# lukebeddow/gripper-mujoco

Hardware: AMD Instinct MI355X
Metric: env-steps/sec (batched rollout) at 4096 envs; obs max-rel-err vs C++ ref (higher is better)
Workload: dtype f64; 1 GPU; C3: set6_synthetic 20 mixed objects, randomised spawn (object drawn per episode, spawn_into_scene grid search on the device), steady state: envs staggered over episode steps 1..250 by an untimed pre-roll, benchmark mix (1 episode in 4: the closed-loop grasp-lift-hold program; otherwise the scripted grasp mix: close / squeeze / palm / lift + jitter), canonical sensor/reward config, device auto-rese; envs_per_gpu=4096, global_envs=4096, parallelism=env-shard x1, substeps_per_env_step=63

## Files before the change

__graft_entry__.py:

```python
from __future__ import annotations

import os
import subprocess
import sys

REPO = os.path.dirname(os.path.abspath(__file__))
PKG = os.path.join(REPO, "gripper-mujoco_amd")


def build() -> None:
    if PKG not in sys.path:
        sys.path.insert(0, PKG)
    from gmx.build import build as build_lib
    build_lib(verbose=True)
    subprocess.run(["make", "-s", "-C", os.path.join(REPO, "oracle"), os.path.join(REPO, "oracle", "liboracle.so")],
                   check=True)
    if os.path.isdir("/root/reference/src"):
        subprocess.run(["make", "-s", "-C", os.path.join(REPO, "oracle"), "ref"], check=True)
    import gmx
    gmx.load_library()


def smoke() -> None:
    import numpy as np
    if PKG not in sys.path:
        sys.path.insert(0, PKG)
    sys.path.insert(0, os.path.join(REPO, "tests"))
    import torch
    assert torch.cuda.is_available(), "smoke() needs a GPU"
    import gmx
    import oracle_lib
    s = gmx.canonical_settings(noise=False, seed=5)
    env = gmx.BatchedGripperEnv(2, object_set="set1_synthetic", settings=s, seed=5, device=0)
    sp = env.make_spawn(x=[0.06, 0.07], y=[0.06, 0.07], idx=0)
    obs0 = env.reset(spawn=sp)
    orc = []
    for e in range(2):
        o = oracle_lib.OracleEnv(env.model, env.cfg, env.objects, e)
        o.reset(sp[e])
        orc.append(o)
        assert np.allclose(obs0[e], o.observation(), atol=1e-5), "reset observation differs from oracle"
    rng = np.random.default_rng(1234)
    for t in range(3):
        a = rng.uniform(-1, 1, size=(2, env.n_actions)).astype(np.float32)
        obs, rew, term, trunc = env.step(a)
        for e in range(2):
            ro, rr, rd = orc[e].step(a[e])
            ro = np.asarray(ro, dtype=np.float64)
            d = np.abs(obs[e] - ro)
            big = np.abs(ro) >= 1e-3
            rel = float((d[big] / np.abs(ro[big])).max()) if big.any() else 0.0
            assert rel <= 1e-4 and float(d[~big].max(initial=0)) <= 1e-4, \
                f"step {t} env {e}: obs rel err {rel:.3e} vs oracle"
            assert bool(term[e]) == bool(rd), "done flag differs from oracle"
            assert abs(float(rew[e]) - float(rr)) <= 1e-5 + 1e-4 * abs(float(rr)), "reward differs from oracle"
    env.close()
    print("smoke ok: 2 envs x 3 env-steps match the oracle")


if __name__ == "__main__":
    build()
    if len(sys.argv) > 1 and sys.argv[1] == "smoke":
        smoke()
```

gripper-mujoco_amd/csrc/gm_newton.hip:

```cpp

#pragma once
#include "gm_rows.h"
#include "gm_newton_point.h"

GM_PHYSICS_BEGIN
template <int CL>
__device__ void smooth_matvec(SharedT<CL>& S, const GmTopo* __restrict__ T, const real* v, real* out, int lane) {
  if (lane < T->nv) {
    const int d = lane, c = T->dof_grp[d], p = T->dof_p[d];
    real acc;
    if (c >= 0 && c < 3) {
      const real* H = S.Hf[c];
      const int f0 = T->dof_f0[c];
      acc = H[TRI(p, 0)] * v[T->dof_base];
#pragma unroll
      for (int j = 1; j <= CL; j++) {
        const real hv = H[(j <= p) ? TRI(p, j) : TRI(j, p)];
        acc = acc + hv * v[f0 + j - 1];
      }
    } else if (c == GM_GRP_BASE) {
      acc = S.Hbb * v[T->dof_base];
#pragma unroll
      for (int f = 0; f < 3; f++)
#pragma unroll
        for (int q = 1; q <= CL; q++) acc = acc + S.Hf[f][TRI(q, 0)] * v[T->dof_f0[f] + q - 1];
      acc = acc + S.Hp[TRI(1, 0)] * v[T->dof_palm];
    } else if (c == GM_GRP_PALM) {
      acc = S.Hp[TRI(1, 0)] * v[T->dof_base] + S.Hp[TRI(1, 1)] * v[T->dof_palm];
    } else {
      acc = 0;
#pragma unroll
      for (int l = 0; l < 6; l++) {
        const real hv = S.Ho[(l <= p) ? TRI(p, l) : TRI(l, p)];
        acc = acc + hv * v[T->dof_obj + l];
      }
    }
    out[d] = acc;
  }
  GM_WAVE_SYNC();
}

struct LineSearch { real alpha; bool capped; };
__device__ __forceinline__ LineSearch line_search(int lane, int ncon, int nl, const RowsT& R, const real* jq, real jql,
                                                  const real* dj, real djl, real g0, real h0, int& nls) {
  const bool clane = lane < ncon;
  real alpha = 1.0, lo = 0.0, hi = 0.0;
  bool hi_set = false, newton = false, have_prev = false;
  unsigned prev = 0;
  int ls = 0;
  for (; ls < GM_NEWTON_MAXLS; ls++) {
    nls++;
    unsigned pat = 0;
    real tg[4], th[4];
#pragma unroll
    for (int e = 0; e < 4; e++) {
      const real j = jq[e] + alpha * dj[e];
      const bool a = clane && j < 0;
      pat |= (unsigned)a << e;
      tg[e] = a ? (R.cD * j) * dj[e] : 0.0;
      th[e] = a ? (R.cD * dj[e]) * dj[e] : 0.0;
    }
    const real jl = jql + alpha * djl;
    const real tgl = (R.lD * jl) * djl, thl = (R.lD * djl) * djl;
    const bool same_piece = have_prev && __ballot(pat != prev) == 0ull;
    if (newton && same_piece) break;
    const real g = (g0 + alpha * h0) + row_sum(lane, ncon, nl, tg, tgl);
    const real hh = h0 + row_sum(lane, ncon, nl, th, thl);
    if (g == 0.0) break;
    if (g < 0) lo = alpha; else { hi = alpha; hi_set = true; }
    if (!(hh > 0)) break;
    real an = alpha - div_n(g, hh);
    newton = true;
    if (!(an > lo) || (hi_set && !(an < hi))) { an = hi_set ? 0.5 * (lo + hi) : 2.0 * alpha; newton = false; }
    prev = pat;
    have_prev = true;
    alpha = an;
  }
  return {alpha, ls == GM_NEWTON_MAXLS};
}

template <int CL, bool CAL, bool DUO = false>
__device__ __forceinline__ void newton_solve(SharedT<CL>& S, const gm_model* __restrict__ m, const GmTopo* __restrict__ T, int lane,
                             bool prof) {
  unsigned long long t0 = prof ? clock64() : 0;
  RowsT R;
  real jq[4], jql;
  bool obj_only;
  constraint_setup<CL, CAL, DUO>(S, m, T, lane, R, jq, jql, obj_only, prof);
  PH(11);
  const int ncon = S.ncon, nl = S.nl, nv = T->nv;
  const bool clane = lane < ncon;
  if (lane < nv) S.qacc[lane] = S.s.qacc_warm[lane];
  GM_WAVE_SYNC();
  PH(12);
  int it = 0, nls = 0;
  bool capped = true;
  bool ls_cap = false;
  const int maxit = (m->newton_maxit > 0 && m->newton_maxit < GM_NEWTON_MAXIT) ? m->newton_maxit : GM_NEWTON_MAXIT;
  for (it = 0; it < maxit; it++) {
    bool act[4];
#pragma unroll
    for (int e = 0; e < 4; e++) act[e] = clane && jq[e] < 0;
    PH(13);
    newton_point<CL>(S, m, T, fresh_lane(), R, act, prof);
    if (prof) t0 = clock64();
    real jx[4], jxl;
    rows_jar<CL>(S, m, T, obj_only, S.xs, lane, R, jx, jxl);
    bool differ = false;
#pragma unroll
    for (int e = 0; e < 4; e++) differ = differ || (clane && ((jx[e] < 0) != act[e]));
    if (__builtin_expect(__ballot(differ) == 0ull, 1)) {
      if (lane < nv) S.qacc[lane] = S.xs[lane];
#pragma unroll
      for (int e = 0; e < 4; e++) jq[e] = jx[e];
      jql = jxl;
      it++;
      capped = false;
      break;
    }
    if (it == 0) smooth_matvec<CL>(S, T, S.qacc, S.Ma, lane);
    if (lane < nv) S.xs[lane] = S.xs[lane] - S.qacc[lane];
    GM_WAVE_SYNC();
    smooth_matvec<CL>(S, T, S.xs, S.Mv, lane);
    const real xl = S.xs[lane];
    const real dd = lane < nv ? xl : 0.0;
    const real g0 = wave_sum(lane < nv ? dd * (S.Ma[lane] - S.frc[lane]) : 0.0);
    const real h0 = wave_sum(lane < nv ? dd * S.Mv[lane] : 0.0);
    real dj[4];
#pragma unroll
    for (int e = 0; e < 4; e++) dj[e] = jx[e] - jq[e];
    const real djl = jxl - jql;
    const LineSearch ls = line_search(lane, ncon, nl, R, jq, jql, dj, djl, g0, h0, nls);
    ls_cap = ls_cap || ls.capped;
    const real alpha = ls.alpha;
    if (lane < nv) {
      S.qacc[lane] = S.qacc[lane] + alpha * S.xs[lane];
      S.Ma[lane] = S.Ma[lane] + alpha * S.Mv[lane];
    }
#pragma unroll
    for (int e = 0; e < 4; e++) jq[e] = jq[e] + alpha * dj[e];
    jql = jql + alpha * djl;
    GM_WAVE_SYNC();
  }
  PH(13);
  if (lane == 0) S.res_valid = capped ? 1 : 0;
  if (capped) {
    RowsT Rc = R;
    bool ac[4];
#pragma unroll
    for (int e = 0; e < 4; e++) { Rc.caref[e] = -jq[e]; ac[e] = clane && jq[e] < 0; }
    Rc.laref = -jql;
    newton_point<CL, true>(S, m, T, fresh_lane(), Rc, ac, false);
    if (lane < nv) S.Mv[lane] = S.Ma[lane] - S.xs[lane];
    GM_WAVE_SYNC();
    if (lane == 0) {
      real A[6][6], x[6];
      for (int k = 0; k < 6; k++)
        for (int l = 0; l <= k; l++) A[k][l] = S.Ho[TRI(k, l)];
      for (int k = 0; k < 6; k++) x[k] = S.Mv[T->dof_obj + k];
      for (int k = 5; k >= 0; k--) {
        const real ik = 1.0 / A[k][k];
        real col[6];
        for (int i = 0; i < k; i++) col[i] = A[k][i];
        for (int i = 0; i < k; i++) {
          const real a = col[i] * ik;
          for (int j = 0; j <= i; j++) A[i][j] = A[i][j] - a * col[j];
          A[k][i] = a;
        }
      }
      for (int k = 5; k >= 0; k--)
        for (int i = 0; i < k; i++) x[i] = x[i] - A[k][i] * x[k];
      for (int k = 0; k < 6; k++) x[k] = x[k] / A[k][k];
      for (int k = 0; k < 6; k++)
        for (int i = 0; i < k; i++) x[k] = x[k] - A[k][i] * x[i];
      for (int k = 0; k < 6; k++) S.Mv[T->dof_obj + k] = x[k];
    }
    GM_WAVE_SYNC();
  }
  real fe[4];
#pragma unroll
  for (int e = 0; e < 4; e++) fe[e] = (clane && jq[e] < 0) ? -(R.cD * jq[e]) : 0.0;
  if (clane) {
    real* C = S.con[lane];
    const real mu = C[10];
    C[11] = ((fe[0] + fe[1]) + fe[2]) + fe[3];
    C[12] = mu * (fe[0] - fe[1]);
    C[13] = mu * (fe[2] - fe[3]);
#pragma unroll
    for (int e = 0; e < 4; e++) S.dbg.efc[nl + 4 * lane + e] = fe[e];
  }
  if (lane < nl) S.dbg.efc[lane] = -(R.lD * jql);
  if (lane < nv) S.s.qacc_warm[lane] = S.qacc[lane];
  if (lane == 0) {
    S.work_nefc += nl + 4 * ncon;
    S.work_newton += it;
    if (capped || ls_cap) S.s.newton_caps += 1;
    if (prof) { S.tph[28] += nl + 4 * ncon; S.tph[30] += it; S.tph[31] += nls; }
  }
  GM_WAVE_SYNC();
}
GM_PHYSICS_END
using gmf::newton_solve;
```

gripper-mujoco_amd/csrc/gm_newton_point.h:

```cpp

#pragma once
#include "gm_rows.h"
#include "gm_arrow.h"

GM_PHYSICS_BEGIN
__device__ __forceinline__ void spatial_K(const real* Q, const real* p, real* K) {
  const real Qm[3][3] = {{Q[0], Q[3], Q[4]}, {Q[3], Q[1], Q[5]}, {Q[4], Q[5], Q[2]}};
  real Bm[3][3];
#pragma unroll
  for (int j = 0; j < 3; j++) {
    real c[3];
    cross3(c, p, Qm[j]);
    Bm[0][j] = c[0]; Bm[1][j] = c[1]; Bm[2][j] = c[2];
  }
  real Am[3][3];
#pragma unroll
  for (int i = 0; i < 3; i++) cross3(Am[i], p, Bm[i]);
  K[0] = Am[0][0]; K[1] = Am[1][1]; K[2] = Am[2][2]; K[3] = Am[0][1]; K[4] = Am[0][2]; K[5] = Am[1][2];
#pragma unroll
  for (int i = 0; i < 3; i++)
#pragma unroll
    for (int j = 0; j < 3; j++) K[6 + 3 * i + j] = Bm[i][j];
#pragma unroll
  for (int k = 0; k < 6; k++) K[15 + k] = Q[k];
}
__device__ __forceinline__ void symK_mul(const real* K, const real* v, real* y) {
  const real *A = K, *B = K + 6, *Q = K + 15;
  const real w0 = v[0], w1 = v[1], w2 = v[2], l0 = v[3], l1 = v[4], l2 = v[5];
  y[0] = A[0] * w0 + A[3] * w1 + A[4] * w2 + B[0] * l0 + B[1] * l1 + B[2] * l2;
  y[1] = A[3] * w0 + A[1] * w1 + A[5] * w2 + B[3] * l0 + B[4] * l1 + B[5] * l2;
  y[2] = A[4] * w0 + A[5] * w1 + A[2] * w2 + B[6] * l0 + B[7] * l1 + B[8] * l2;
  y[3] = B[0] * w0 + B[3] * w1 + B[6] * w2 + Q[0] * l0 + Q[3] * l1 + Q[4] * l2;
  y[4] = B[1] * w0 + B[4] * w1 + B[7] * w2 + Q[3] * l0 + Q[1] * l1 + Q[5] * l2;
  y[5] = B[2] * w0 + B[5] * w1 + B[8] * w2 + Q[4] * l0 + Q[5] * l1 + Q[2] * l2;
}

__device__ __forceinline__ void contact_composite(const real* qf, const real* pos, real* Kc, real* Fs) {
  spatial_K(qf, pos, Kc);
  cross3(Fs, pos, qf + 6);
  Fs[3] = qf[6]; Fs[4] = qf[7]; Fs[5] = qf[8];
}
template <int CL>
__device__ __forceinline__ void composite_add(const SharedT<CL>& S, int c, int b, real* K, real* F) {
  const real* qf = S.nw.QF[c];
  const real pos[3] = {S.con[c][1], S.con[c][2], S.con[c][3]};
  const real sg = (S.cbody[c][1] == b) ? 1.0 : -1.0;
  real Kc[21], Fs[6];
  contact_composite(qf, pos, Kc, Fs);
#pragma unroll
  for (int k = 0; k < 21; k++) K[k] += Kc[k];
#pragma unroll
  for (int k = 0; k < 6; k++) F[k] += sg * Fs[k];
}
template <int CL, class Col>
__device__ __forceinline__ void object_columns(const SharedT<CL>& S, const GmTopo* T, Col col) {
#pragma unroll
  for (int k0 = 0; k0 < 6; k0 += 3) {
    real co[18];
#pragma unroll
    for (int k = 0; k < 3; k++)
#pragma unroll
      for (int t = 0; t < 6; t++) co[6 * k + t] = S.cdof[T->dof_obj + k0 + k][t];
    keep_n<18>(co);
#pragma unroll
    for (int k = 0; k < 3; k++) col(k0 + k, co + 6 * k);
  }
}
template <int CL>
__device__ __forceinline__ void newton_contact_qf(SharedT<CL>& S, int lane, int ncon, const RowsT& R, const bool* act,
                                                  real (&Q)[6], real (&F)[3]) {
#pragma unroll
  for (int k = 0; k < 6; k++) Q[k] = 0;
#pragma unroll
  for (int k = 0; k < 3; k++) F[k] = 0;
  if (lane < ncon) {
    const real* C = S.con[lane];
    real t2[3];
    cross3(t2, C + 4, C + 7);
#pragma unroll
    for (int ed = 0; ed < 4; ed++) {
      real u[3];
      edge_dir(C, t2, ed, u);
      const real w = act[ed] ? R.cD : 0.0;
      const real du[3] = {w * u[0], w * u[1], w * u[2]};
      Q[0] += du[0] * u[0]; Q[1] += du[1] * u[1]; Q[2] += du[2] * u[2];
      Q[3] += du[0] * u[1]; Q[4] += du[0] * u[2]; Q[5] += du[1] * u[2];
      const real g = w * R.caref[ed];
      F[0] += g * u[0]; F[1] += g * u[1]; F[2] += g * u[2];
    }
    real* qf = S.nw.QF[lane];
#pragma unroll
    for (int k = 0; k < 6; k++) qf[k] = Q[k];
    qf[6] = F[0]; qf[7] = F[1]; qf[8] = F[2];
  }
  GM_WAVE_SYNC();
}

template <int CL>
__device__ __forceinline__ void newton_ground_composites(SharedT<CL>& S, const GmTopo* T, int lane, int ncon,
                                                         const real (&Q)[6], const real (&F)[3]) {
  static_assert(sizeof(S.st.root) >= sizeof(real) * 8 * 27, "ground composites: eight contacts per round in the chain-root stage");
  real (*gs)[27] = reinterpret_cast<real (*)[27]>(&S.st.root[0][0]);
  const int pr = T->pair_gobj;
  int c0 = 0, c1 = 0;
  if (pr >= 0) {
    c0 = __builtin_amdgcn_readfirstlane((int)S.pair_off[pr]);
    c1 = c0 + __builtin_amdgcn_readfirstlane((int)S.pair_cnt[pr]);
    if (c1 > ncon) c1 = ncon;
  }
  real gacc = 0;
  for (int r0 = c0; r0 < c1; r0 += 8) {
    if (r0 > c0) GM_WAVE_SYNC();
    if (lane >= r0 && lane < r0 + 8 && lane < c1) {
      const real qf[9] = {Q[0], Q[1], Q[2], Q[3], Q[4], Q[5], F[0], F[1], F[2]};
      const real pos[3] = {S.con[lane][1], S.con[lane][2], S.con[lane][3]};
      const real sg = (S.cbody[lane][1] == T->body_obj) ? 1.0 : -1.0;
      real Kc[21], Fs[6];
      contact_composite(qf, pos, Kc, Fs);
      real* g = gs[lane - r0];
#pragma unroll
      for (int k = 0; k < 21; k++) g[k] = Kc[k];
#pragma unroll
      for (int k = 0; k < 6; k++) g[21 + k] = sg * Fs[k];
    }
    GM_WAVE_SYNC();
    if (lane < 27) {
      real v[8];
#pragma unroll
      for (int j = 0; j < 8; j++) v[j] = gs[j][lane];
      keep_n<8>(v);
#pragma unroll
      for (int j = 0; j < 8; j++) gacc = (r0 + j < c1) ? gacc + v[j] : gacc;
    }
  }
  if (lane < 27) S.go[lane] = gacc;
}

template <int CL>
__device__ __forceinline__ void newton_schur(SharedT<CL>& S, int lane) {
  if (lane < 28) {
    int i = 0;
#pragma unroll
    for (int t = 1; t < 7; t++) i += (lane >= t * (t + 1) / 2) ? 1 : 0;
    const int j = lane - i * (i + 1) / 2;
    real acc[3];
    border_transfer_sums<CL>(S, i, [&](int f, int k1) { return S.fs.lbub[f][k1][7 + j]; }, acc);
    real v = S.fs.bbx[lane];
    v = (((v - acc[0]) - acc[1]) - acc[2]) - S.fs.plb[i] * S.fs.plb[7 + j];
    S.fs.bbx[lane] = v;
  }
}

template <int CL>
__device__ __forceinline__ void newton_border_factor(SharedT<CL>& S, int lane, real (&hb)[7], real& invd) {
  const int bi = lane - 48;
  const bool border = lane >= 48 && lane < 55;
  if (border) {
#pragma unroll
    for (int j = 0; j < 7; j++)
      if (j <= bi) hb[j] = S.fs.bbx[bi * (bi + 1) / 2 + j];
#pragma unroll
    for (int k = 6; k >= 0; k--) {
      const real ihk = rcp_piv(row_bcast(hb[k], k));
      real bk[7];
#pragma unroll
      for (int j = 0; j < k; j++) bk[j] = row_bcast(hb[j], k);
      const bool upd = bi < k, piv = bi == k;
      real Bik = 0.0;
#pragma unroll
      for (int j = 0; j < k; j++) Bik = (bi == j) ? bk[j] : Bik;
      const real a = Bik * ihk;
      const real aa = upd ? a : 0.0;
#pragma unroll
      for (int j = 0; j < k; j++) hb[j] = hb[j] - bk[j] * aa;
      hb[k] = upd ? a : hb[k];
      invd = piv ? ihk : invd;
    }
#pragma unroll
    for (int j = 0; j < 6; j++) hb[j] = (j < bi) ? hb[j] * invd : hb[j];
  }
}

template <int CL>
__device__ __forceinline__ void newton_backsolve(SharedT<CL>& S, const GmTopo* T, int lane,
                                                 const real (&h)[CL + 1], const real (&hb)[7], real rhs, real invd) {
  const int rowf = lane >> 4, p = lane & 15, bi = lane - 48;
  const bool border = (lane >= 48 && lane < 55);
  real y = rhs;
  if (lane < 48) {
    y = chain_forward<CL>(y, h, p);
    if ((rowf < 3 && p >= 1 && p <= CL)) S.fs.ych[rowf][p - 1] = y;
  } else if (lane == GM_LANE_PALM_F) {
    S.fs.ypalm = y;
  }
  GM_WAVE_SYNC();
  if (border) {
    real acc[3];
    border_transfer_sums<CL>(S, bi, [&](int f, int k1) { return S.fs.ych[f][k1]; }, acc);
    y = (((y - acc[0]) - acc[1]) - acc[2]) - S.fs.plb[bi] * S.fs.ypalm;
#pragma unroll
    for (int k = 6; k >= 0; k--) {
      const real yk = row_bcast(y, k);
      const real Lc = (bi < k) ? hb[k] : 0.0;
      y = y - Lc * yk;
    }
  }
  y = y * invd;
  if (border) {
#pragma unroll
    for (int j = 0; j < 6; j++) {
      const real xj = row_bcast(y, j);
      const real Lr = (j < bi) ? hb[j] : 0.0;
      y = y - Lr * xj;
    }
  }
  real xb[7];
#pragma unroll
  for (int t = 0; t < 7; t++) xb[t] = readlane_real(y, 48 + t);
  if (lane < 48) {
#pragma unroll
    for (int t = 0; t < 7; t++) y = y - hb[t] * xb[t];
    y = chain_backward<CL>(y, h, p);
    if ((rowf < 3 && p >= 1 && p <= CL)) S.xs[T->dof_f0[rowf] + p - 1] = y;
  } else if (lane == GM_LANE_PALM_F) {
#pragma unroll
    for (int t = 0; t < 7; t++) y = y - hb[t] * xb[t];
    S.xs[T->dof_palm] = y;
  } else if (border) {
    S.xs[bi == 0 ? T->dof_base : T->dof_obj + bi - 1] = y;
  }
  GM_WAVE_SYNC();
}

template <int CL, bool RHS_ONLY = false>
__device__ void newton_point(SharedT<CL>& S, const gm_model* __restrict__ m, const GmTopo* __restrict__ T, int lane,
                             const RowsT& R, const bool* act, bool prof) {
  unsigned long long t0 = prof ? clock64() : 0;
  const int ncon = S.ncon, nl = S.nl;
  real Q[6], F[3];
  newton_contact_qf<CL>(S, lane, ncon, R, act, Q, F);
  newton_ground_composites<CL>(S, T, lane, ncon, Q, F);
  const int b = T->lane_body[lane];
  real Ko[21], Fo[6];
#pragma unroll
  for (int k = 0; k < 21; k++) Ko[k] = 0;
#pragma unroll
  for (int k = 0; k < 6; k++) Fo[k] = 0;
  bool have_g = false;
  int cs[2] = {0, 0}, ns[2] = {0, 0};
#pragma unroll
  for (int s = 0; s < 2; s++) {
    const int pr = T->lane_opair[lane][s];
    const int pg = T->lane_gpair[lane][s];
    if (pg >= 0 && S.pair_cnt[pg] > 0 && S.pair_off[pg] < ncon) have_g = true;
    if (pr >= 0) {
      const int c0 = S.pair_off[pr];
      int c1 = c0 + S.pair_cnt[pr];
      if (c1 > ncon) c1 = ncon;
      cs[s] = c0;
      ns[s] = c1 > c0 ? c1 - c0 : 0;
    }
  }
  const bool have_o = ns[0] + ns[1] > 0;
  {
    for (int t = 0; t < ns[0] + ns[1]; t++) {
      const int c = t < ns[0] ? cs[0] + t : cs[1] + (t - ns[0]);
      composite_add<CL>(S, c, b, Ko, Fo);
    }
  }
  const bool any_g = __ballot(have_g) != 0ull;
  const bool any_o = __ballot(have_o) != 0ull;
  PH(3);
  if (any_o) {
#pragma unroll
    for (int off = 1; off < CL; off <<= 1) {
#pragma unroll
      for (int k = 0; k < 21; k++) Ko[k] += row_shl(Ko[k], off);
#pragma unroll
      for (int k = 0; k < 6; k++) Fo[k] += row_shl(Fo[k], off);
    }
  }
  {
    const int root = (lane == 1) ? 0 : (lane == 17) ? 1 : (lane == 33) ? 2 : (lane == 49) ? 3 : -1;
    if (root >= 0) {
      real* st = S.st.root[root];
#pragma unroll
      for (int k = 0; k < 21; k++) st[k] = Ko[k];
#pragma unroll
      for (int k = 0; k < 6; k++) st[42 + k] = Fo[k];
    }
  }
  GM_WAVE_SYNC();
  if (lane < 27) {
    const int k = lane < 21 ? lane : 42 + lane - 21;
    real acc = 0;
#pragma unroll
    for (int c = 0; c < 4; c++) acc += S.st.root[c][k];
    S.st.comp[k] = acc;
  }
  GM_WAVE_SYNC();
  if (lane < 27) {
    S.st.oo[lane] = (lane < 21) ? S.st.comp[lane] + S.go[lane] : S.go[lane] - S.st.comp[42 + lane - 21];
  }
  GM_WAVE_SYNC();
  PH(4);
  real h[CL + 1], hb[7], rhs = 0;
#pragma unroll
  for (int j = 0; j <= CL; j++) h[j] = 0;
#pragma unroll
  for (int k = 0; k < 7; k++) hb[k] = 0;
  const int rowf = lane >> 4, p = lane & 15;
  const real* cdb = S.cdof[T->dof_base];
  if (rowf < 3 && p >= 1 && p <= CL) {
    const int d = T->dof_f0[rowf] + p - 1;
    const real* H = S.Hf[rowf];
    if (any_o) {
      real cd[6], y[6], Hr[CL + 1];
#pragma unroll
      for (int k = 0; k < 6; k++) cd[k] = S.cdof[d][k];
#pragma unroll
      for (int j = 0; j <= CL; j++) Hr[j] = H[TRI(p, j)];
      keep_n<CL + 1>(Hr);
      symK_mul(Ko, cd, y);
#pragma unroll
      for (int j = 1; j <= CL; j++) {
        real cj[6];
#pragma unroll
        for (int k = 0; k < 6; k++) cj[k] = row_bcast(cd[k], j);
        const real v = Hr[j] + dot6(cj, y);
        keep(v);
        h[j] = (j <= p) ? v : h[j];
      }
      hb[0] = Hr[0] + dot6(cdb, y);
      object_columns<CL>(S, T, [&](int l, const real* co) { hb[1 + l] = -dot6(co, y); });
      rhs = S.frc[d] + dot6(cd, Fo);
    } else {
      real Hr[CL + 1];
#pragma unroll
      for (int j = 0; j <= CL; j++) Hr[j] = H[TRI(p, j)];
      keep_n<CL + 1>(Hr);
#pragma unroll
      for (int j = 1; j <= CL; j++) h[j] = (j <= p) ? Hr[j] : h[j];
      hb[0] = Hr[0];
      rhs = S.frc[d];
    }
  } else if (lane == GM_LANE_PALM_F && !any_o) {
    h[1] = S.Hp[TRI(1, 1)];
    hb[0] = S.Hp[TRI(1, 0)];
    rhs = S.frc[T->dof_palm];
  } else if (lane == GM_LANE_PALM_F) {
    const int d = T->dof_palm;
    const real* st = S.st.root[3];
    real K0[27], y[6];
#pragma unroll
    for (int k = 0; k < 21; k++) K0[k] = st[k];
#pragma unroll
    for (int k = 0; k < 6; k++) K0[21 + k] = S.cdof[d][k];
    keep_n<27>(K0);
    const real* cd = K0 + 21;
    symK_mul(K0, cd, y);
    h[1] = S.Hp[TRI(1, 1)] + dot6(cd, y);
    hb[0] = S.Hp[TRI(1, 0)] + dot6(cdb, y);
    object_columns<CL>(S, T, [&](int l, const real* co) { hb[1 + l] = -dot6(co, y); });
    rhs = S.frc[d] + dot6(cd, st + 42);
  } else if (lane >= 48 && lane < 55) {
    const int i = lane - 48;
    const real* cp = S.st.comp;
    real yob[6] = {0, 0, 0, 0, 0, 0};
    if (any_o) {
      real KBo[21];
#pragma unroll
      for (int k = 0; k < 21; k++) KBo[k] = cp[k];
      keep_n<21>(KBo);
      symK_mul(KBo, cdb, yob);
    }
    if (i == 0) {
      hb[0] = any_o ? S.Hbb + dot6(cdb, yob) : S.Hbb;
      rhs = any_o ? S.frc[T->dof_base] + dot6(cdb, cp + 42) : S.frc[T->dof_base];
    } else {
      const int k = i - 1;
      real KC[27], yk[6];
#pragma unroll
      for (int t = 0; t < 21; t++) KC[t] = S.st.oo[t];
#pragma unroll
      for (int t = 0; t < 6; t++) KC[21 + t] = S.cdof[T->dof_obj + k][t];
      keep_n<27>(KC);
      const real* cok = KC + 21;
      symK_mul(KC, cok, yk);
      hb[0] = -dot6(cok, yob);
      object_columns<CL>(S, T, [&](int l, const real* co) {
        const real v = S.Ho[TRI(k, l)] + dot6(co, yk);
        keep(v);
        hb[1 + l] = (l <= k) ? v : hb[1 + l];
      });
      rhs = S.frc[T->dof_obj + k] + dot6(cok, S.st.oo + 21);
    }
  }
  if (__builtin_expect(any_g, 0)) {
    real Kg[21], Fg[6];
#pragma unroll
    for (int k = 0; k < 21; k++) Kg[k] = 0;
#pragma unroll
    for (int k = 0; k < 6; k++) Fg[k] = 0;
#pragma unroll
    for (int s = 0; s < 2; s++) {
      const int pr = T->lane_gpair[lane][s];
      if (pr < 0) continue;
      const int c0 = S.pair_off[pr];
      int c1 = c0 + S.pair_cnt[pr];
      if (c1 > ncon) c1 = ncon;
      for (int c = c0; c < c1; c++) {
        composite_add<CL>(S, c, b, Kg, Fg);
      }
    }
#pragma unroll
    for (int off = 1; off < CL; off <<= 1) {
#pragma unroll
      for (int k = 0; k < 21; k++) Kg[k] += row_shl(Kg[k], off);
#pragma unroll
      for (int k = 0; k < 6; k++) Fg[k] += row_shl(Fg[k], off);
    }
    const int root = (lane == 1) ? 0 : (lane == 17) ? 1 : (lane == 33) ? 2 : (lane == 49) ? 3 : -1;
    if (root >= 0) {
      real* st = S.st.root[root];
#pragma unroll
      for (int k = 0; k < 21; k++) st[21 + k] = Kg[k];
#pragma unroll
      for (int k = 0; k < 6; k++) st[48 + k] = Fg[k];
    }
    GM_WAVE_SYNC();
    const bool chainrow = rowf < 3 && p >= 1 && p <= CL;
    if (lane == GM_LANE_PALM_F) {
#pragma unroll
      for (int k = 0; k < 21; k++) Kg[k] = S.st.root[3][21 + k];
#pragma unroll
      for (int k = 0; k < 6; k++) Fg[k] = S.st.root[3][48 + k];
    } else if (lane == 48) {
#pragma unroll
      for (int k = 0; k < 21; k++) Kg[k] = ((S.st.root[0][21 + k] + S.st.root[1][21 + k]) + S.st.root[2][21 + k]) + S.st.root[3][21 + k];
#pragma unroll
      for (int k = 0; k < 6; k++) Fg[k] = ((S.st.root[0][48 + k] + S.st.root[1][48 + k]) + S.st.root[2][48 + k]) + S.st.root[3][48 + k];
    }
    if (chainrow || lane == GM_LANE_PALM_F || lane == 48) {
      const int d = chainrow ? T->dof_f0[rowf] + p - 1 : lane == 48 ? T->dof_base : T->dof_palm;
      real cd[6], yg[6];
#pragma unroll
      for (int k = 0; k < 6; k++) cd[k] = S.cdof[d][k];
      symK_mul(Kg, cd, yg);
      if (chainrow) {
#pragma unroll
        for (int j = 1; j <= CL; j++)
          if (j <= p) h[j] += dot6(S.cdof[T->dof_f0[rowf] + j - 1], yg);
      } else if (lane == GM_LANE_PALM_F) {
        h[1] += dot6(cd, yg);
      }
      hb[0] += dot6(cdb, yg);
      rhs += dot6(cd, Fg);
    }
  }
  for (int r = 0; r < nl; r++) {
    const int d = __builtin_amdgcn_readlane(R.ldof, r);
    const real lD = readlane_real(R.lD, r), lR = readlane_real(R.lD * R.laref, r);
    if (T->dof_grp[d] < 3) {
      const int f = T->dof_grp[d], pd = T->dof_p[d];
      if (rowf == f && p == pd) {
#pragma unroll
        for (int j = 1; j <= CL; j++) if (j == pd) h[j] += lD;
        rhs += lR;
      }
    } else if (lane == GM_LANE_PALM_F) {
      h[1] += lD;
      rhs += lR;
    }
  }
  if constexpr (RHS_ONLY) {
    if (rowf < 3 && p >= 1 && p <= CL) S.xs[T->dof_f0[rowf] + p - 1] = rhs;
    else if (lane == GM_LANE_PALM_F) S.xs[T->dof_palm] = rhs;
    else if (lane >= 48 && lane < 55) S.xs[lane == 48 ? T->dof_base : T->dof_obj + lane - 49] = rhs;
    GM_WAVE_SYNC();
    return;
  }
  GM_WAVE_SYNC();
  PH(7);
  real invd = 1.0;
  if (lane < 48) {
#pragma unroll
    for (int k = CL; k >= 1; k--) {
      const real hkk = row_bcast(h[k], k);
      const real ihk = rcp_piv(hkk);
      real hk[CL + 1], hkb[7];
#pragma unroll
      for (int j = 1; j < k; j++) hk[j] = row_bcast(h[j], k);
#pragma unroll
      for (int t = 0; t < 7; t++) hkb[t] = row_bcast(hb[t], k);
      const bool upd = p >= 1 && p < k, piv = p == k;
      real Hpk = 0.0;
#pragma unroll
      for (int j = 1; j < k; j++) Hpk = (p == j) ? hk[j] : Hpk;
      const real a = Hpk * ihk;
      const real aa = upd ? a : 0.0;
      if (piv && rowf < 3) {
        real* ub = S.fs.lbub[rowf][k - 1] + 7;
#pragma unroll
        for (int t = 0; t < 7; t++) ub[t] = hb[t];
      }
#pragma unroll
      for (int j = 1; j < k; j++) h[j] = h[j] - hk[j] * aa;
#pragma unroll
      for (int t = 0; t < 7; t++) hb[t] = hb[t] - hkb[t] * aa;
      h[k] = upd ? a : h[k];
      invd = piv ? ihk : invd;
    }
#pragma unroll
    for (int j = 1; j < CL; j++) h[j] = (j < p) ? h[j] * invd : h[j];
#pragma unroll
    for (int t = 0; t < 7; t++) hb[t] = hb[t] * invd;
    if (rowf < 3 && p >= 1 && p <= CL) {
      real* lb = S.fs.lbub[rowf][p - 1];
#pragma unroll
      for (int t = 0; t < 7; t++) lb[t] = hb[t];
    }
  } else if (lane == GM_LANE_PALM_F) {
    const real ih = rcp_piv(h[1]);
    real* pl = S.fs.plb;
#pragma unroll
    for (int t = 0; t < 7; t++) { pl[7 + t] = hb[t]; hb[t] = hb[t] * ih; pl[t] = hb[t]; }
    invd = ih;
  } else if (lane >= 48 && lane < 55) {
    const int i = lane - 48;
#pragma unroll
    for (int j = 0; j < 7; j++)
      if (j <= i) S.fs.bbx[i * (i + 1) / 2 + j] = hb[j];
  }
  GM_WAVE_SYNC();
  newton_schur<CL>(S, lane);
  GM_WAVE_SYNC();
  newton_border_factor<CL>(S, lane, hb, invd);
  PH(14);
  newton_backsolve<CL>(S, T, lane, h, hb, rhs, invd);
  PH(24);
}
GM_PHYSICS_END
```

gripper-mujoco_amd/gmx/build.py:

```python
from __future__ import annotations

import os
import subprocess

from ._lib import PKG_DIR, REPO_DIR, LIB_PATH

SOURCES = ["csrc/gm_capi.hip", "csrc/gm_calib.hip", "csrc/gm_host_model.cpp", "csrc/gm_mjcf.cpp"]
HIPCC = os.environ.get("HIPCC", "/opt/rocm/bin/hipcc")
FLAGS = ["--offload-arch=gfx950", "-O3", "-std=c++17", "-fPIC",
         "-fhip-fp32-correctly-rounded-divide-sqrt", "-munsafe-fp-atomics",
         "-ffp-contract=off",
         "-mllvm", "-disable-machine-licm"]


def build(verbose: bool = False, force: bool = False, out: str | None = None, extra_flags=()) -> str:
    lib_path = out or LIB_PATH
    srcs = [os.path.join(PKG_DIR, s) for s in SOURCES]
    csrc = os.path.join(PKG_DIR, "csrc")
    deps = sorted(set(srcs + [os.path.join(csrc, f) for f in os.listdir(csrc) if f.endswith((".hip", ".h", ".inc"))])) + \
        [os.path.join(REPO_DIR, "include", f) for f in ("gripper_mi355x.h", "gm_settings.def")]
    if not force and out is None and os.path.exists(LIB_PATH):
        t = os.path.getmtime(LIB_PATH)
        if all(os.path.getmtime(d) <= t for d in deps):
            return LIB_PATH
    objdir = os.path.join(os.path.dirname(LIB_PATH), "obj" if out is None else "obj_" + os.path.basename(out))
    os.makedirs(objdir, exist_ok=True)
    inc = ["-I" + os.path.join(REPO_DIR, "include"), "-I" + os.path.join(PKG_DIR, "csrc")]
    procs, objs = [], []
    headers = [os.path.join(csrc, "gm_state.h")] + \
        [os.path.join(REPO_DIR, "include", f) for f in ("gripper_mi355x.h", "gm_settings.def")]
    for src in srcs:
        obj = os.path.join(objdir, os.path.basename(src) + ".o")
        objs.append(obj)
        tu_deps = [src] + headers if src.endswith(".cpp") else deps
        if not force and os.path.exists(obj) and all(os.path.getmtime(d) <= os.path.getmtime(obj) for d in tu_deps):
            continue
        cmd = [HIPCC, *FLAGS, *extra_flags, *inc, "-c", src, "-o", obj]
        if verbose:
            print(" ".join(cmd))
        procs.append((subprocess.Popen(cmd), cmd))
    for p, cmd in procs:
        if p.wait() != 0:
            raise subprocess.CalledProcessError(p.returncode, cmd)
    link = [HIPCC, "--offload-arch=gfx950", "-shared", "-fPIC", *objs, "-o", lib_path + ".tmp"]
    if verbose:
        print(" ".join(link))
    subprocess.run(link, check=True)
    os.replace(lib_path + ".tmp", lib_path)
    return lib_path
```

gripper-mujoco_amd/gmx/env.py:

```python
from __future__ import annotations

import ctypes as C

import numpy as np

from ._lib import (GM_MAX_CON, GM_MAX_DOF, GM_MAX_EFC, load_library, ModelBlob, ConfigBlob, ModelParams, Spawn, SpawnParams, make_object_set,
                   BINARY_EVENTS, LINEAR_EVENTS, RolloutParams)
from .settings import canonical_settings, MAX_EPISODE_STEPS


_M64 = np.uint64(0xFFFFFFFFFFFFFFFF)


def _splitmix64(x):
    x = (x + np.uint64(0x9E3779B97F4A7C15)) & _M64
    x = ((x ^ (x >> np.uint64(30))) * np.uint64(0xBF58476D1CE4E5B9)) & _M64
    x = ((x ^ (x >> np.uint64(27))) * np.uint64(0x94D049BB133111EB)) & _M64
    return x ^ (x >> np.uint64(31))


def spawn_int(seed, gid, episode, k, lo, hi):
    with np.errstate(over="ignore"):
        gid = np.asarray(gid, dtype=np.int64).astype(np.uint64)
        ep = np.asarray(episode, dtype=np.int64).astype(np.uint32).astype(np.uint64)
        kk = np.asarray(k, dtype=np.int64).astype(np.uint64)
        x = (np.uint64(seed) + gid * np.uint64(0xD1B54A32D192ED03) + ep * np.uint64(0x8CB92BA72F3D8DD7)
             + kk * np.uint64(0x9E3779B97F4A7C15)) & _M64
        h = _splitmix64(x)
        span = np.uint64(hi - lo + 1)
        return lo + (((h >> np.uint64(32)) * span) >> np.uint64(32)).astype(np.int64)


def random_fractions(seed, gid, episode, step, n_actions):
    with np.errstate(over="ignore"):
        gid = np.asarray(gid, dtype=np.int64).astype(np.uint64).reshape(-1, 1)
        ep = np.asarray(episode, dtype=np.int64).astype(np.uint32).astype(np.uint64).reshape(-1, 1)
        kk = np.asarray(step, dtype=np.int64).astype(np.uint32).astype(np.uint64).reshape(-1, 1)
        ii = np.arange(n_actions, dtype=np.uint64).reshape(1, -1)
        x = (np.uint64(seed) * np.uint64(0xA24BAED4963EE407) + gid * np.uint64(0xD1B54A32D192ED03)
             + ep * np.uint64(0x8CB92BA72F3D8DD7) + kk * np.uint64(0x9E3779B97F4A7C15)
             + ii * np.uint64(0xF1357AEA2E62A9C5)) & _M64
        h = _splitmix64(x)
        return ((h >> np.uint64(40)).astype(np.float32) * np.float32(2.0 / 16777216.0) - np.float32(1.0)).astype(np.float32)


def spawn_draws(seed, gids, episodes, n_objects, position_noise_mm: int = 10, rotation_noise_deg: int = 5):
    nm, nd = int(position_noise_mm), int(rotation_noise_deg)
    idx = spawn_int(seed, gids, episodes, 0, 0, n_objects - 1)
    x = spawn_int(seed, gids, episodes, 1, -nm, nm) * 1e-3
    y = spawn_int(seed, gids, episodes, 2, -nm, nm) * 1e-3
    noise = spawn_int(seed, gids, episodes, 3, -nd, nd)
    opt = spawn_int(seed, gids, episodes, 4, 0, 2)
    rot = (60 * opt + noise) * (np.pi / 180.0)
    return idx, x, y, rot


class BatchedGripperEnv:
    def __init__(self, n_envs: int, object_set: str = "set6_synthetic", settings=None,
                 model_params: ModelParams | None = None, device: int = 0, seed: int = 1234,
                 env_offset: int = 0, max_episode_steps: int = MAX_EPISODE_STEPS, lib=None,
                 model_blob: ModelBlob | None = None, objects=None):
        self.lib = lib if lib is not None else load_library()
        self.n_envs = int(n_envs)
        self.model = model_blob if model_blob is not None else ModelBlob(model_params)
        self.settings = settings if settings is not None else canonical_settings(seed=seed)
        self.cfg = ConfigBlob(self.settings, self.model)
        self.objects = objects if objects is not None else make_object_set(object_set, seed)
        self.max_episode_steps = max_episode_steps
        self.device = device
        self.seed = int(seed)
        self.env_offset = int(env_offset)
        self._episode = np.zeros(self.n_envs, dtype=np.int64)
        self._ctx = C.c_void_p()
        rc = self.lib.gm_create(self.model.ptr, self.cfg.ptr, self.objects, len(self.objects), self.n_envs,
                                int(env_offset), int(device), int(seed), C.byref(self._ctx))
        if rc != 0:
            msg = self.lib.gm_last_error(self._ctx).decode() if self._ctx else ""
            raise RuntimeError(f"gm_create failed ({rc}) {msg}")
        self._check(self.lib.gm_set_random_spawn(self._ctx, 1, self.seed, 10, 5))
        self.n_obs = self.lib.gm_n_obs(self._ctx)
        self.n_actions = self.lib.gm_n_actions(self._ctx)
        self.current_step = np.zeros(self.n_envs, dtype=np.int64)
        self._obs = np.zeros((self.n_envs, self.n_obs), dtype=np.float32)
        self._rew = np.zeros(self.n_envs, dtype=np.float32)
        self._done = np.zeros(self.n_envs, dtype=np.uint8)

    def _check(self, rc):
        if rc != 0:
            raise RuntimeError(self.lib.gm_last_error(self._ctx).decode() or f"gm error {rc}")

    def close(self):
        if self._ctx:
            self.lib.gm_destroy(self._ctx)
            self._ctx = C.c_void_p()

    def __del__(self):
        try:
            self.close()
        except Exception:
            pass

    @property
    def ctx(self):
        return self._ctx

    @property
    def stream(self) -> int:
        return self.lib.gm_stream(self._ctx)

    def make_spawn(self, mask=None, idx=None, x=None, y=None, rot=None):
        n = self.n_envs
        gids = self.env_offset + np.arange(n)
        self._sync_episode()
        si, sx, sy, sr = spawn_draws(self.seed, gids, self._episode + 1, len(self.objects))
        if idx is not None: si = np.broadcast_to(np.asarray(idx), (n,))
        if x is not None: sx = np.broadcast_to(np.asarray(x, dtype=np.float64), (n,))
        if y is not None: sy = np.broadcast_to(np.asarray(y, dtype=np.float64), (n,))
        if rot is not None: sr = np.broadcast_to(np.asarray(rot, dtype=np.float64), (n,))
        arr = (Spawn * n)()
        for e in range(n):
            arr[e].object_index = int(si[e]); arr[e].x = float(sx[e]); arr[e].y = float(sy[e]); arr[e].zrot = float(sr[e])
        return arr

    def _sync_episode(self):
        from ._lib import env_state_view
        self._episode[:] = env_state_view(self.env_states())["episode"]

    def reset(self, mask=None, spawn=None):
        if mask is not None:
            m = np.ascontiguousarray(np.asarray(mask, dtype=np.uint8))
            self._check(self.lib.gm_reset(self._ctx, m.ctypes.data_as(C.POINTER(C.c_uint8)), spawn))
            self.current_step[m.astype(bool)] = 0
            self._episode[m.astype(bool)] += 1
        else:
            self._check(self.lib.gm_reset(self._ctx, None, spawn))
            self.current_step[:] = 0
            self._episode += 1
        return self.observation()

    def spawn_into_scene(self, params, mask=None):
        if isinstance(params, SpawnParams):
            arr, n = (SpawnParams * 1)(params), 1
        else:
            arr = (SpawnParams * len(params))(*params)
            n = len(params)
        ok = np.zeros(self.n_envs, dtype=np.uint8)
        m = None
        if mask is not None:
            m = np.ascontiguousarray(np.asarray(mask, dtype=np.uint8))
        self._check(self.lib.gm_spawn_into_scene(self._ctx, None if m is None else m.ctypes.data_as(C.POINTER(C.c_uint8)),
                                                 arr, n, ok.ctypes.data_as(C.POINTER(C.c_uint8))))
        return ok.astype(bool)

    def set_scene_spawn(self, params, max_tries: int = 3):
        self._check(self.lib.gm_set_scene_spawn(self._ctx, None if params is None else C.byref(params), int(max_tries)))

    def scripted_actions(self, seed: int, jitter: float = 0.2) -> np.ndarray:
        out = np.zeros((self.n_envs, self.n_actions), dtype=np.float32)
        self._check(self.lib.gm_scripted_actions(self._ctx, int(seed), float(jitter), out.ctypes.data, 0))
        return out

    def program_actions(self, seed: int = 0, jitter: float = 0.2, mode: int = 3) -> np.ndarray:
        out = np.zeros((self.n_envs, self.n_actions), dtype=np.float32)
        self._check(self.lib.gm_program_actions(self._ctx, int(seed), float(jitter), int(mode), out.ctypes.data, 0))
        return out

    def set_action(self, actions):
        a = np.ascontiguousarray(np.asarray(actions, dtype=np.float32).reshape(self.n_envs, self.n_actions))
        self._check(self.lib.gm_set_action(self._ctx, a.ctypes.data, 0))

    def set_discrete_action(self, actions):
        a = np.ascontiguousarray(np.asarray(actions, dtype=np.int32).reshape(self.n_envs))
        self._check(self.lib.gm_set_discrete_action(self._ctx, a.ctypes.data, 0))

    def action_step(self):
        self._check(self.lib.gm_step(self._ctx))

    def rollout(self, n_steps: int, action_mode: int = 0, seed: int = 1234, jitter: float = 0.2,
                max_episode_steps: int | None = None, records_dev_ptr: int | None = None):
        mx = self.max_episode_steps if max_episode_steps is None else max_episode_steps
        p = RolloutParams()
        p.action_mode, p.max_episode_steps, p.seed, p.jitter = int(action_mode), int(mx), int(seed), float(jitter)
        self._check(self.lib.gm_rollout(self._ctx, int(n_steps), C.byref(p), C.c_void_p(records_dev_ptr or 0)))

    def set_motor_target(self, xyz, mask=None):
        t = np.ascontiguousarray(np.asarray(xyz, dtype=np.float64).reshape(-1, 3))
        if t.shape[0] not in (1, self.n_envs):
            raise ValueError(f"xyz must be 3 values or [{self.n_envs}, 3]")
        ok = np.ones(self.n_envs, dtype=np.uint8)
        m = None if mask is None else np.ascontiguousarray(np.asarray(mask, dtype=np.uint8).reshape(self.n_envs))
        self._check(self.lib.gm_set_motor_target(self._ctx, None if m is None else m.ctypes.data, t.ctypes.data,
                                                 t.shape[0], ok.ctypes.data))
        return ok.astype(bool)

    def sensor_si(self):
        out = np.zeros((self.n_envs, 5), dtype=np.float32)
        self._check(self.lib.gm_get_sensor_si(self._ctx, out.ctypes.data))
        return out

    def observation(self):
        self._check(self.lib.gm_get_obs(self._ctx, self._obs.ctypes.data, 0))
        return self._obs.copy()

    def outputs(self):
        self._check(self.lib.gm_get_outputs(self._ctx, self._obs.ctypes.data, self._rew.ctypes.data,
                                            self._done.ctypes.data))
        return self._obs.copy(), self._rew.copy(), self._done.astype(bool)

    def reward_done(self):
        self._check(self.lib.gm_get_reward_done(self._ctx, self._rew.ctypes.data, self._done.ctypes.data, 0))
        return self._rew.copy(), self._done.astype(bool)

    def step(self, actions, discrete: bool = False):
        self.current_step += 1
        if discrete:
            self.set_discrete_action(actions)
        else:
            self.set_action(actions)
        self.action_step()
        obs, rew, term = self.outputs()
        trunc = self.current_step >= self.max_episode_steps
        term = np.where(trunc, False, term)
        return obs, rew, term, trunc

    def step_device(self, actions_dev_ptr: int):
        self._check(self.lib.gm_set_action(self._ctx, C.c_void_p(actions_dev_ptr), 1))
        self._check(self.lib.gm_step(self._ctx))

    def set_stream(self, stream_handle: int | None):
        self._check(self.lib.gm_set_stream(self._ctx, C.c_void_p(stream_handle or 0)))

    def upload_spawn(self, spawn):
        import torch
        raw = np.frombuffer(bytes(spawn), dtype=np.uint8)
        self._spawn_dev = torch.from_numpy(raw.copy()).to(f"cuda:{self.device}")
        return self._spawn_dev.data_ptr()

    def autoreset_device(self, spawn_dev_ptr: int, returns_dev_ptr: int | None = None,
                         max_episode_steps: int | None = None, episodes_dev_ptr: int | None = None):
        mx = self.max_episode_steps if max_episode_steps is None else max_episode_steps
        self._check(self.lib.gm_autoreset_episodes(self._ctx, int(mx), C.c_void_p(spawn_dev_ptr), 1,
                                                   C.c_void_p(returns_dev_ptr or 0),
                                                   C.c_void_p(episodes_dev_ptr or 0)))

    def device_buffers(self):
        return (self.lib.gm_device_obs(self._ctx), self.lib.gm_device_reward(self._ctx),
                self.lib.gm_device_done(self._ctx))

    def last_step_ms(self) -> float:
        v = C.c_float()
        self._check(self.lib.gm_last_step_ms(self._ctx, C.byref(v)))
        return float(v.value)

    def chunk_stats(self) -> dict:
        v = (C.c_uint32 * 7)()
        t = (C.c_uint64 * 5)()
        self._check(self.lib.gm_chunk_stats(self._ctx, v, t))
        span = (t[2] - t[0]) * 1e-5 if t[2] > t[0] else 0.0
        return dict(started=v[0], finished=v[1], yields=v[2], resumes=v[3], every=v[4], workgroups=v[5], steals=v[6],
                    span_ms=span, fresh_empty_ms=(t[1] - t[0]) * 1e-5 if t[1] >= t[0] and span else 0.0,
                    busy=(t[3] / (v[5] * (t[2] - t[0]))) if span and v[5] else 0.0,
                    poll=(t[4] / (v[5] * (t[2] - t[0]))) if span and v[5] else 0.0)

    def claim_waits(self) -> dict:
        v = (C.c_uint32 * 2)()
        self._check(self.lib.gm_chunk_claim_waits(self._ctx, v))
        return dict(waiting_claims=int(v[0]), polls=int(v[1]))

    def job_stats(self):
        import numpy as np
        clk = np.zeros(self.n_envs, dtype=np.uint32)
        yl = np.zeros(self.n_envs, dtype=np.int32)
        self._check(self.lib.gm_chunk_job_stats(self._ctx, clk.ctypes.data_as(C.c_void_p),
                                                 yl.ctypes.data_as(C.c_void_p)))
        return clk, yl

    def chunk_timeline(self):
        import numpy as np
        info = self.dispatch_info()
        G = info["grid"]
        buf = (C.c_uint64 * max(1, G + 2 * self.n_envs))()
        n = self.lib.gm_chunk_timeline(self._ctx, buf, G + 2 * self.n_envs)
        if n < 0:
            raise RuntimeError(f"gm_chunk_timeline failed ({n})")
        t = (C.c_uint64 * 5)()
        v = (C.c_uint32 * 7)()
        self._check(self.lib.gm_chunk_stats(self._ctx, v, t))
        raw = np.frombuffer(buf, dtype=np.uint64, count=n)
        wg = raw[:G]
        ends = ((wg & np.uint64((1 << 60) - 1)).astype(np.float64) - float(t[0])) * 1e-5
        ev = (raw[G:].astype(np.float64).reshape(-1, 2) - float(t[0])) * 1e-5
        return ends, (wg >> np.uint64(60)).astype(np.int32), ev

    def dispatch_info(self) -> dict:
        v = (C.c_int32 * 4)()
        self._check(self.lib.gm_dispatch_info(self._ctx, v))
        return dict(chunk=v[0], grid=v[1], waves_per_env=v[2], last_launch_env_steps=v[3])

    def state(self):
        q = np.zeros((self.n_envs, self.model.nq), dtype=np.float64)
        v = np.zeros((self.n_envs, self.model.nv), dtype=np.float64)
        t = np.zeros(self.n_envs, dtype=np.float64)
        self._check(self.lib.gm_get_state(self._ctx, q.ctypes.data_as(C.POINTER(C.c_double)),
                                          v.ctypes.data_as(C.POINTER(C.c_double)),
                                          t.ctypes.data_as(C.POINTER(C.c_double))))
        return q, v, t

    def set_state(self, qpos, qvel):
        q = np.ascontiguousarray(np.asarray(qpos, dtype=np.float64))
        v = np.ascontiguousarray(np.asarray(qvel, dtype=np.float64))
        self._check(self.lib.gm_set_state(self._ctx, q.ctypes.data_as(C.POINTER(C.c_double)),
                                          v.ctypes.data_as(C.POINTER(C.c_double))))

    def env_states(self) -> np.ndarray:
        sz = int(self.lib.gm_env_state_size())
        out = np.zeros((self.n_envs, sz), dtype=np.uint8)
        self._check(self.lib.gm_get_env_states(self._ctx, out.ctypes.data))
        return out

    def set_env_states(self, states):
        a = np.ascontiguousarray(np.asarray(states, dtype=np.uint8))
        if a.shape != (self.n_envs, int(self.lib.gm_env_state_size())):
            raise ValueError(f"expected {(self.n_envs, int(self.lib.gm_env_state_size()))} state records, got {a.shape}")
        self._check(self.lib.gm_set_env_states(self._ctx, a.ctypes.data))

    def target(self):
        e = np.zeros((self.n_envs, 4)); es = np.zeros((self.n_envs, 3), dtype=np.int32)
        ns = np.zeros((self.n_envs, 3), dtype=np.int32); b = np.zeros((self.n_envs, 3))
        self._check(self.lib.gm_get_target(self._ctx, e.ctypes.data_as(C.POINTER(C.c_double)),
                                           es.ctypes.data_as(C.POINTER(C.c_int32)),
                                           ns.ctypes.data_as(C.POINTER(C.c_int32)),
                                           b.ctypes.data_as(C.POINTER(C.c_double))))
        return e, es, ns, b

    def event_rows(self):
        W = len(BINARY_EVENTS) + len(LINEAR_EVENTS)
        rows = np.zeros((self.n_envs, W), dtype=np.int32)
        absc = np.zeros((self.n_envs, W), dtype=np.int32)
        lastv = np.zeros((self.n_envs, W), dtype=np.float32)
        self._check(self.lib.gm_get_event_rows(self._ctx, rows.ctypes.data_as(C.POINTER(C.c_int32)),
                                               absc.ctypes.data_as(C.POINTER(C.c_int32)),
                                               lastv.ctypes.data_as(C.POINTER(C.c_float))))
        return rows, absc, lastv

    def overflow(self):
        o = np.zeros(self.n_envs, dtype=np.int32)
        self._check(self.lib.gm_get_overflow(self._ctx, o.ctypes.data_as(C.POINTER(C.c_int32))))
        return o

    def debug_substep(self, full: bool = False):
        n = self.n_envs
        ncon = np.zeros(n, dtype=np.int32)
        nefc = np.zeros(n, dtype=np.int32)
        con = np.zeros((n, GM_MAX_CON, 16), dtype=np.float64)
        f = np.zeros((n, GM_MAX_EFC), dtype=np.float64)
        qacc = np.zeros((n, GM_MAX_DOF), dtype=np.float64)
        w = np.zeros((n, 6), dtype=np.float64)
        d = C.POINTER(C.c_double)
        self._check(self.lib.gm_debug_substep(self._ctx, ncon.ctypes.data_as(C.POINTER(C.c_int32)),
                                              con.ctypes.data_as(d), f.ctypes.data_as(d), qacc.ctypes.data_as(d),
                                              nefc.ctypes.data_as(C.POINTER(C.c_int32)), w.ctypes.data_as(d)))
        if full:
            return ncon, con, f, qacc, nefc, w
        return ncon, con, f, qacc

    PHASES = ("kinematics", "crb_rne", "mass_forces", "  n:QF+bodies", "  n:scans+composites", "collision",
              "newton_solve", "  n:H_assembly", "integrate", "update_all", "monitor_sensors",
              "  n:setup", "  n:warm_start", "  n:jar+line_search", "  n:factor", "  k:A_hinge", "  k:B_chains",
              "  crb:chains", "e:sense", "e:update_env", "e:get_obs", "e:done_reward", "substep_body", "env_step",
              "  n:solve", "t:start", "t:end", "cu")
    PH_NEFC, PH_MPR, PH_NEWTON, PH_LS = 28, 29, 30, 31
    N_PHASE = 32

    def step_profiled(self):
        ph = np.zeros((self.n_envs, self.N_PHASE), dtype=np.uint64)
        self._check(self.lib.gm_step_profiled(self._ctx, ph.ctypes.data_as(C.POINTER(C.c_uint64))))
        return ph
```

Before: 736,900 env-steps/s.

## Add decoupled Newton point solve for object-only contact on first iteration

When every active contact touches only the object (obj_only, uniform across the wave), the first Newton iteration uses a specialised factorisation. It eliminates the finger chains onto a border block made of the base and the object's six DOFs, instead of the general coupled factorisation. The aim is to shorten the dense Hessian factor and solve on that common path. It adds a second code path with signed-zero bookkeeping to keep results bitwise consistent, plus an A/B build flag and a profiling counter; register pressure may rise in the solver.

```diff
diff --git a/__graft_entry__.py b/__graft_entry__.py
--- a/__graft_entry__.py
+++ b/__graft_entry__.py
@@ -11,8 +11,22 @@
 def build() -> None:
     if PKG not in sys.path:
         sys.path.insert(0, PKG)
-    from gmx.build import build as build_lib
+    import threading
+    from gmx.build import build as build_lib, build_no_decoupled
+    failed = []
+
+    def build_ab():
+        try:
+            build_no_decoupled()
+        except Exception as e:
+            failed.append(e)
+
+    ab = threading.Thread(target=build_ab)
+    ab.start()
     build_lib(verbose=True)
+    ab.join()
+    if failed:
+        raise failed[0]
     subprocess.run(["make", "-s", "-C", os.path.join(REPO, "oracle"), os.path.join(REPO, "oracle", "liboracle.so")],
                    check=True)
     if os.path.isdir("/root/reference/src"):
diff --git a/gripper-mujoco_amd/csrc/gm_newton.hip b/gripper-mujoco_amd/csrc/gm_newton.hip
--- a/gripper-mujoco_amd/csrc/gm_newton.hip
+++ b/gripper-mujoco_amd/csrc/gm_newton.hip
@@ -87,6 +87,9 @@
   real jq[4], jql;
   bool obj_only;
   constraint_setup<CL, CAL, DUO>(S, m, T, lane, R, jq, jql, obj_only, prof);
+#ifndef GM_NO_DECOUPLED_POINT
+  const bool decoupled = __builtin_amdgcn_readfirstlane((int)obj_only) != 0;
+#endif
   PH(11);
   const int ncon = S.ncon, nl = S.nl, nv = T->nv;
   const bool clane = lane < ncon;
@@ -102,6 +105,12 @@
 #pragma unroll
     for (int e = 0; e < 4; e++) act[e] = clane && jq[e] < 0;
     PH(13);
+#ifndef GM_NO_DECOUPLED_POINT
+    if (it == 0 && decoupled) {
+      newton_point_decoupled<CL>(S, m, T, fresh_lane(), R, act, prof);
+      if (prof && lane == 0) S.tph[27] += 1ull << 32;
+    } else
+#endif
     newton_point<CL>(S, m, T, fresh_lane(), R, act, prof);
     if (prof) t0 = clock64();
     real jx[4], jxl;
diff --git a/gripper-mujoco_amd/csrc/gm_newton_point.h b/gripper-mujoco_amd/csrc/gm_newton_point.h
--- a/gripper-mujoco_amd/csrc/gm_newton_point.h
+++ b/gripper-mujoco_amd/csrc/gm_newton_point.h
@@ -540,4 +540,183 @@
   newton_backsolve<CL>(S, T, lane, h, hb, rhs, invd);
   PH(24);
 }
+
+#ifndef GM_NO_DECOUPLED_POINT
+template <int CL>
+__device__ void newton_point_decoupled(SharedT<CL>& S, const gm_model* __restrict__ m, const GmTopo* __restrict__ T, int lane,
+                                       const RowsT& R, const bool* act, bool prof) {
+  static_assert(CL >= 7, "the object's six columns sit in h[1..6] and ride on pivots 6 .. 1");
+  unsigned long long t0 = prof ? clock64() : 0;
+  const int ncon = S.ncon, nl = S.nl;
+  real Q[6], F[3];
+  newton_contact_qf<CL>(S, lane, ncon, R, act, Q, F);
+  newton_ground_composites<CL>(S, T, lane, ncon, Q, F);
+  PH(3);
+  GM_WAVE_SYNC();
+  PH(4);
+  real h[CL + 1], hb0 = 0, rhs = 0;
+#pragma unroll
+  for (int j = 0; j <= CL; j++) h[j] = 0;
+  const int rowf = lane >> 4, p = lane & 15;
+  const bool chainrow = rowf < 3 && p >= 1 && p <= CL;
+  const bool border = lane >= 48 && lane < 55;
+  if (chainrow) {
+    const int d = T->dof_f0[rowf] + p - 1;
+    const real* H = S.Hf[rowf];
+    real Hr[CL + 1];
+#pragma unroll
+    for (int j = 0; j <= CL; j++) Hr[j] = H[TRI(p, j)];
+    keep_n<CL + 1>(Hr);
+#pragma unroll
+    for (int j = 1; j <= CL; j++) h[j] = (j <= p) ? Hr[j] : h[j];
+    hb0 = Hr[0];
+    rhs = S.frc[d];
+  } else if (lane == GM_LANE_PALM_F) {
+    h[1] = S.Hp[TRI(1, 1)];
+    hb0 = S.Hp[TRI(1, 0)];
+    rhs = S.frc[T->dof_palm];
+  } else if (lane == 48) {
+    hb0 = S.Hbb;
+    rhs = S.frc[T->dof_base];
+  } else if (border) {
+    const int k = lane - 49;
+    const real yob[6] = {0, 0, 0, 0, 0, 0};
+    real KC[27], yk[6];
+#pragma unroll
+    for (int t = 0; t < 21; t++) KC[t] = S.go[t];
+#pragma unroll
+    for (int t = 0; t < 6; t++) KC[21 + t] = S.cdof[T->dof_obj + k][t];
+    keep_n<27>(KC);
+    const real* cok = KC + 21;
+    symK_mul(KC, cok, yk);
+    hb0 = -dot6(cok, yob);
+    hb0 = hb0 - 0.0 * S.Hp[TRI(1, 0)];
+    object_columns<CL>(S, T, [&](int l, const real* co) {
+      const real v = S.Ho[TRI(k, l)] + dot6(co, yk);
+      keep(v);
+      h[1 + l] = (l <= k) ? v : h[1 + l];
+    });
+    rhs = S.frc[T->dof_obj + k] + dot6(cok, S.go + 21);
+  }
+  for (int r = 0; r < nl; r++) {
+    const int d = __builtin_amdgcn_readlane(R.ldof, r);
+    const real lD = readlane_real(R.lD, r), lR = readlane_real(R.lD * R.laref, r);
+    if (T->dof_grp[d] < 3) {
+      const int f = T->dof_grp[d], pd = T->dof_p[d];
+      if (rowf == f && p == pd) {
+#pragma unroll
+        for (int j = 1; j <= CL; j++) if (j == pd) h[j] += lD;
+        rhs += lR;
+      }
+    } else if (lane == GM_LANE_PALM_F) {
+      h[1] += lD;
+      rhs += lR;
+    }
+  }
+  PH(7);
+  real invd = 1.0, sacc = 0.0;
+  const real pub = readlane_real(hb0, GM_LANE_PALM_F), ypalm = readlane_real(rhs, GM_LANE_PALM_F);
+  const real pih = rcp_piv(readlane_real(h[1], GM_LANE_PALM_F));
+  const real plb = pub * pih;
+#define GM_DEC_PIVOT(ROW3) do { \
+    const real hkk = row_bcast(h[k], k); \
+    const real ihk = rcp_piv(hkk); \
+    real hk[CL + 1]; \
+    _Pragma("unroll") for (int j = 1; j < k; j++) hk[j] = row_bcast(h[j], k); \
+    const real hkb = row_bcast(hb0, k); \
+    const bool upd = ((ROW3) && rowf == 3) ? p < k : (p >= 1 && p < k); \
+    const bool piv = p == k; \
+    real Hpk = ((ROW3) && lane == 48) ? hkb : 0.0; \
+    _Pragma("unroll") for (int j = 1; j < k; j++) Hpk = (p == j) ? hk[j] : Hpk; \
+    const real a = Hpk * ihk; \
+    const real aa = upd ? a : 0.0; \
+    const real lbk = hkb * ihk; \
+    sacc = sacc + lbk * hkb; \
+    _Pragma("unroll") for (int j = 1; j < k; j++) h[j] = h[j] - hk[j] * aa; \
+    hb0 = hb0 - hkb * aa; \
+    h[k] = upd ? a : h[k]; \
+    invd = piv ? ihk : invd; \
+  } while (0)
+  if (lane < 48) {
+#pragma unroll
+    for (int k = CL; k >= 7; k--) GM_DEC_PIVOT(false);
+  }
+  if (lane < 55) {
+#pragma unroll
+    for (int k = 6; k >= 1; k--) GM_DEC_PIVOT(true);
+#pragma unroll
+    for (int j = 1; j < CL; j++) h[j] = (j < p) ? h[j] * invd : h[j];
+    hb0 = (lane == 48) ? hb0 : hb0 * invd;
+  } else if (lane == GM_LANE_PALM_F) {
+    hb0 = hb0 * pih;
+    invd = pih;
+  }
+#undef GM_DEC_PIVOT
+  const real sa0 = readlane_real(sacc, 1), sa1 = readlane_real(sacc, 17), sa2 = readlane_real(sacc, 33);
+  if (lane == 48) {
+    hb0 = (((hb0 - sa0) - sa1) - sa2) - plb * pub;
+    invd = rcp_piv(hb0);
+  }
+  PH(14);
+  real y = rhs, facc = 0.0;
+  if (border) y = (lane == 48) ? -0.0 : y - 0.0 * ypalm;
+#define GM_DEC_FORWARD(ROW3) do { \
+    const real yk = row_bcast(y, k); \
+    const real lbk = row_bcast(hb0, k); \
+    facc = facc + lbk * yk; \
+    const bool upd = ((ROW3) && rowf == 3) ? p < k : (p >= 1 && p < k); \
+    const real Lc = upd ? h[k] : 0.0; \
+    y = y - Lc * yk; \
+  } while (0)
+  if (lane < 48) {
+#pragma unroll
+    for (int k = CL; k >= 7; k--) GM_DEC_FORWARD(false);
+  }
+  if (lane < 55) {
+#pragma unroll
+    for (int k = 6; k >= 1; k--) GM_DEC_FORWARD(true);
+  }
+#undef GM_DEC_FORWARD
+  const real fa0 = readlane_real(facc, 1), fa1 = readlane_real(facc, 17), fa2 = readlane_real(facc, 33);
+  if (lane == 48) {
+    const real Y = (((rhs - fa0) - fa1) - fa2) - plb * ypalm;
+    y = Y + y;
+  }
+  const real yb6 = readlane_real(y, 48);
+  if (border) y = y - 0.0 * yb6;
+  y = y * invd;
+  const real tb = readlane_real(y, 48);
+  if (border) {
+    const real Lr0 = (lane > 48) ? hb0 : 0.0;
+    y = y - Lr0 * tb;
+#pragma unroll
+    for (int j = 1; j < 6; j++) {
+      const real xj = row_bcast(y, j);
+      const real Lr = (j < p) ? h[j] : 0.0;
+      y = y - Lr * xj;
+    }
+  }
+  real xb[7];
+#pragma unroll
+  for (int t = 0; t < 7; t++) xb[t] = readlane_real(y, 48 + t);
+  bool neg = false;
+#pragma unroll
+  for (int t = 1; t < 7; t++) neg = neg || __double_as_longlong(xb[t]) < 0;
+  const real zsub = neg ? -0.0 : 0.0;
+  if (lane < 48) {
+    y = y - hb0 * xb[0];
+    y = y - zsub;
+    y = chain_backward<CL>(y, h, p);
+    if (chainrow) S.xs[T->dof_f0[rowf] + p - 1] = y;
+  } else if (lane == GM_LANE_PALM_F) {
+    y = y - hb0 * xb[0];
+    y = y - zsub;
+    S.xs[T->dof_palm] = y;
+  } else if (border) {
+    S.xs[lane == 48 ? T->dof_base : T->dof_obj + lane - 49] = y;
+  }
+  GM_WAVE_SYNC();
+  PH(24);
+}
+#endif
 GM_PHYSICS_END
diff --git a/gripper-mujoco_amd/gmx/build.py b/gripper-mujoco_amd/gmx/build.py
--- a/gripper-mujoco_amd/gmx/build.py
+++ b/gripper-mujoco_amd/gmx/build.py
@@ -11,6 +11,24 @@
          "-fhip-fp32-correctly-rounded-divide-sqrt", "-munsafe-fp-atomics",
          "-ffp-contract=off",
          "-mllvm", "-disable-machine-licm"]
+
+
+NO_DECOUPLED_LIB = os.path.join(os.path.dirname(LIB_PATH), "libgm_no_decoupled.so")
+
+
+def _deps():
+    csrc = os.path.join(PKG_DIR, "csrc")
+    return sorted(os.path.join(PKG_DIR, s) for s in SOURCES) + \
+        sorted(os.path.join(csrc, f) for f in os.listdir(csrc) if f.endswith((".hip", ".h", ".inc"))) + \
+        [os.path.join(REPO_DIR, "include", f) for f in ("gripper_mi355x.h", "gm_settings.def")]
+
+
+def build_no_decoupled(verbose: bool = False) -> str:
+    if os.path.exists(NO_DECOUPLED_LIB):
+        t = os.path.getmtime(NO_DECOUPLED_LIB)
+        if all(os.path.getmtime(d) <= t for d in _deps()):
+            return NO_DECOUPLED_LIB
+    return build(verbose=verbose, out=NO_DECOUPLED_LIB, extra_flags=["-DGM_NO_DECOUPLED_POINT"])
 
 
 def build(verbose: bool = False, force: bool = False, out: str | None = None, extra_flags=()) -> str:
diff --git a/gripper-mujoco_amd/gmx/env.py b/gripper-mujoco_amd/gmx/env.py
--- a/gripper-mujoco_amd/gmx/env.py
+++ b/gripper-mujoco_amd/gmx/env.py
@@ -375,4 +375,6 @@
     def step_profiled(self):
         ph = np.zeros((self.n_envs, self.N_PHASE), dtype=np.uint64)
         self._check(self.lib.gm_step_profiled(self._ctx, ph.ctypes.data_as(C.POINTER(C.c_uint64))))
+        self.decoupled_points = (ph[:, 27] >> np.uint64(32)).astype(np.int64)
+        ph[:, 27] &= np.uint64(0xFFFFFFFF)
         return ph
```

Measured after the change: 776,200 env-steps/s (median of 6 runs). 5.3% higher.
